# weimengmeng1999/AdapterSIS

Hardware: AMD Instinct MI355X
Metric: training images/sec, ViT-L/14 588^2 adapter fine-tune (higher is better)
Workload: dtype f16; 1 GPU; vit_large/14 frozen + CAViT/CACNN adapters (n_last_blocks=4) + FeatureDecoder, 588x588, batch 12/GPU, reference_exact train.py step (fwd + decoder bwd + all-reduce + SGD), random-init weights; global_batch=12, image_size=588, parallelism=dp1, split_precision_convs=True, split_attn_out=False, precise_level=0, fold_attn_scale=True, fused_qkv=False, dead_cacnn_elided=True, c1_elided=True, ln_fold=True, mx_conv=True, mx_dense=True, conv_halo=True, fuse_cls_up=False, skipped_optimizer_steps=0

## Files before the change

adaptersis_amd/csrc/convhalo.hip:

```cpp
#include <type_traits>
#include "asis_common.h"

namespace {

typedef int v4i_ __attribute__((ext_vector_type(4)));
typedef int v8i_ __attribute__((ext_vector_type(8)));

template <int COUT>
__global__ __launch_bounds__(256, 2) void conv_halo_mx_kernel(const f16* __restrict__ x_hi, const f16* __restrict__ x_mx,
                                                              const f16* __restrict__ w_hi, const f16* __restrict__ w_mx,
                                                              const float* __restrict__ bias, const float* __restrict__ amax_a,
                                                              const float* __restrict__ amax_b, float* __restrict__ out,
                                                              float* __restrict__ stats, int B, int H, int W, int Cin, int TH, int TW, int CT) {
  constexpr int NB = COUT / 16;
  constexpr int MB = 4;
  constexpr int HP = 18 * 18;
  constexpr int HALO = HP * 64;
  constexpr int WT = COUT * 64;
  constexpr int NT = 256;
  __shared__ __attribute__((aligned(16))) f16 lds[HALO + 3 * WT];
  f16* const halo = lds;
  f16* const wbuf0 = lds + HALO;

  const int tid = threadIdx.x, lane = tid & 63;
  const int wid = __builtin_amdgcn_readfirstlane(tid >> 6);
  const int r16 = lane & 15, q16 = lane >> 4;
  int bid = blockIdx.x;
  const int tx_ = bid % TW; bid /= TW;
  const int ty_ = bid % TH;
  const int b = bid / TH;
  const int y0 = ty_ * 16, x0 = tx_ * 16;
  const int64_t img = (int64_t)b * H * W;
  const int K9 = 9 * Cin;
  const int mx_sc = mx_code<f16>(*amax_a, *amax_b);
  const int mx_one = 127;
  const int n0 = blockIdx.y * COUT;
  w_hi += (int64_t)n0 * K9;
  w_mx += (int64_t)n0 * K9;

  f32x4 acc[MB][NB];
#pragma unroll
  for (int i = 0; i < MB; ++i)
#pragma unroll
    for (int j = 0; j < NB; ++j) acc[i][j] = f32x4{0.f, 0.f, 0.f, 0.f};

  const int ngroups = (Cin / 64) * 2;
  constexpr int HLOADS = (HP * 8 + NT - 1) / NT;
  uint4 hreg[HLOADS];
  auto halo_load = [&](int g) {
    const f16* src = (g & 1) ? x_mx : x_hi;
    const int c0 = (g >> 1) * 64;
#pragma unroll
    for (int it = 0; it < HLOADS; ++it) {
      int idx = it * NT + tid;
      idx = idx < HP * 8 ? idx : HP * 8 - 1;
      const int p = idx >> 3, ch = idx & 7;
      const int hy = p / 18, hx = p - hy * 18;
      const int gy = y0 - 1 + hy, gx = x0 - 1 + hx;
      const bool ok = (unsigned)gy < (unsigned)H && (unsigned)gx < (unsigned)W;
      const int cy = ok ? gy : 0, cx = ok ? gx : 0;
      const uint4 v = *reinterpret_cast<const uint4*>(src + ((img + (int64_t)cy * W + cx) * Cin + c0 + ch * 8));
      hreg[it] = ok ? v : make_uint4(0u, 0u, 0u, 0u);
    }
  };
  auto halo_store = [&]() {
#pragma unroll
    for (int it = 0; it < HLOADS; ++it) {
      const int idx = it * NT + tid;
      if (idx < HP * 8) {
        const int p = idx >> 3, ch = idx & 7;
        *reinterpret_cast<uint4*>(halo + p * 64 + ((ch ^ ((p >> 1) & 7)) << 3)) = hreg[it];
      }
    }
  };
  typedef __attribute__((address_space(3))) void* lds_ptr;
  typedef const __attribute__((address_space(1))) void* glb_ptr;
  static_assert(COUT == 64, "two DMA pieces per wave and tap: 4 waves x 2 x 8 rows");
  auto w_dma = [&](int st) {
    const int g = st / 9, tap = st - g * 9;
    const f16* src = (g & 1) ? w_mx : w_hi;
    const int c0 = (g >> 1) * 64;
    f16* dst = wbuf0 + (st % 3) * WT;
#pragma unroll
    for (int i = 0; i < 2; ++i) {
      const int q = wid * 2 + i;
      const int n = q * 8 + (lane >> 3), ch = (lane & 7) ^ ((n >> 1) & 7);
      __builtin_amdgcn_global_load_lds((glb_ptr)(src + (int64_t)n * K9 + tap * Cin + c0 + ch * 8), (lds_ptr)(dst + q * 8 * 64), 16, 0, 0);
    }
  };
  auto mfma_mx = [](f32x4& a, v8i_ x, v8i_ y, int sx, int sy) {
    asm volatile("v_mfma_scale_f32_16x16x128_f8f6f4 %0, %1, %2, %0, %3, %4 op_sel_hi:[0,0,0]" : "+v"(a) : "v"(x), "v"(y), "v"(sx), "v"(sy));
  };

  const int nsteps = ngroups * 9;
  w_dma(0);
  w_dma(1);
  halo_load(0);
  halo_store();
  asm volatile("s_waitcnt vmcnt(0)" ::: "memory");
  __syncthreads();

  int step = 0;
  for (int g = 0; g < ngroups; ++g) {
    const bool next_group = g + 1 < ngroups;
#pragma unroll 1
   for (int tap = 0; tap < 9; ++tap, ++step) {
    if (step + 2 < nsteps) w_dma(step + 2);
    if (tap == 0 && next_group) halo_load(g + 1);
    const f16* wt = wbuf0 + (step % 3) * WT;
    const int ty = tap / 3, tx = tap - ty * 3;
    v8i_ aw[MB];
#pragma unroll
    for (int mb = 0; mb < MB; ++mb) {
      const int p = (wid * MB + mb + ty) * 18 + r16 + tx;
      aw[mb] = __builtin_shufflevector(*reinterpret_cast<const v4i_*>(halo + p * 64 + (((q16) ^ ((p >> 1) & 7)) << 3)),
                                       *reinterpret_cast<const v4i_*>(halo + p * 64 + (((4 + q16) ^ ((p >> 1) & 7)) << 3)), 0, 1, 2, 3, 4, 5, 6, 7);
    }
    auto lo4 = [](v8i_ x) { return __builtin_bit_cast(f16x8, __builtin_shufflevector(x, x, 0, 1, 2, 3)); };
    auto hi4 = [](v8i_ x) { return __builtin_bit_cast(f16x8, __builtin_shufflevector(x, x, 4, 5, 6, 7)); };
    constexpr int NH = 2;
#pragma unroll
    for (int h = 0; h < NB / NH; ++h) {
      v8i_ bw[NH];
#pragma unroll
      for (int k = 0; k < NH; ++k) {
        const int n = (h * NH + k) * 16 + r16;
        bw[k] = __builtin_shufflevector(*reinterpret_cast<const v4i_*>(wt + n * 64 + (((q16) ^ ((n >> 1) & 7)) << 3)),
                                        *reinterpret_cast<const v4i_*>(wt + n * 64 + (((4 + q16) ^ ((n >> 1) & 7)) << 3)), 0, 1, 2, 3, 4, 5, 6, 7);
      }
      if (g & 1) {
        asm volatile("s_waitcnt lgkmcnt(0)" ::: "memory");
#pragma unroll
        for (int k = 0; k < NH; ++k)
#pragma unroll
          for (int mb = 0; mb < MB; ++mb) mfma_mx(acc[mb][h * NH + k], bw[k], aw[mb], mx_sc, mx_one);
      } else {
#pragma unroll
        for (int k = 0; k < NH; ++k)
#pragma unroll
          for (int mb = 0; mb < MB; ++mb) {
            acc[mb][h * NH + k] = T16<f16>::mfma16(lo4(bw[k]), lo4(aw[mb]), acc[mb][h * NH + k]);
            acc[mb][h * NH + k] = T16<f16>::mfma16(hi4(bw[k]), hi4(aw[mb]), acc[mb][h * NH + k]);
          }
      }
    }
    if (step + 1 < nsteps) {
      if (step + 2 >= nsteps) asm volatile("s_waitcnt vmcnt(0)" ::: "memory");
      else if (tap == 0 && next_group) asm volatile("s_waitcnt vmcnt(13)" ::: "memory");
      else asm volatile("s_waitcnt vmcnt(2)" ::: "memory");
    }
    __syncthreads();
    if (tap == 8 && next_group) {
      halo_store();
      __syncthreads();
    }
   }
  }

  float4 s_sum[NB], s_sq[NB];
#pragma unroll
  for (int nb = 0; nb < NB; ++nb) {
    s_sum[nb] = make_float4(0.f, 0.f, 0.f, 0.f);
    s_sq[nb] = make_float4(0.f, 0.f, 0.f, 0.f);
  }
#pragma unroll
  for (int mb = 0; mb < MB; ++mb) {
    const int gy = y0 + wid * MB + mb, gx = x0 + r16;
    const bool ok = gy < H && gx < W;
    float* op = out + (img + (int64_t)(ok ? gy : 0) * W + (ok ? gx : 0)) * CT + n0;
#pragma unroll
    for (int nb = 0; nb < NB; ++nb) {
      const int n = nb * 16 + 4 * q16;
      const float4 bv = bias ? *reinterpret_cast<const float4*>(bias + n0 + n) : make_float4(0.f, 0.f, 0.f, 0.f);
      const float4 v = make_float4(acc[mb][nb][0] + bv.x, acc[mb][nb][1] + bv.y, acc[mb][nb][2] + bv.z, acc[mb][nb][3] + bv.w);
      if (ok) {
        *reinterpret_cast<float4*>(op + n) = v;
        s_sum[nb].x += v.x; s_sum[nb].y += v.y; s_sum[nb].z += v.z; s_sum[nb].w += v.w;
        s_sq[nb].x += v.x * v.x; s_sq[nb].y += v.y * v.y; s_sq[nb].z += v.z * v.z; s_sq[nb].w += v.w * v.w;
      }
    }
  }
  if (stats) {
#pragma unroll
    for (int nb = 0; nb < NB; ++nb)
#pragma unroll
      for (int o = 1; o < 16; o <<= 1) {
        s_sum[nb].x += __shfl_xor(s_sum[nb].x, o, 64); s_sum[nb].y += __shfl_xor(s_sum[nb].y, o, 64);
        s_sum[nb].z += __shfl_xor(s_sum[nb].z, o, 64); s_sum[nb].w += __shfl_xor(s_sum[nb].w, o, 64);
        s_sq[nb].x += __shfl_xor(s_sq[nb].x, o, 64); s_sq[nb].y += __shfl_xor(s_sq[nb].y, o, 64);
        s_sq[nb].z += __shfl_xor(s_sq[nb].z, o, 64); s_sq[nb].w += __shfl_xor(s_sq[nb].w, o, 64);
      }
    float* red = reinterpret_cast<float*>(lds);
    if (r16 == 0) {
#pragma unroll
      for (int nb = 0; nb < NB; ++nb) {
        *reinterpret_cast<float4*>(red + (wid * 2 + 0) * COUT + nb * 16 + 4 * q16) = s_sum[nb];
        *reinterpret_cast<float4*>(red + (wid * 2 + 1) * COUT + nb * 16 + 4 * q16) = s_sq[nb];
      }
    }
    __syncthreads();
    if (tid < 2 * COUT) {
      const int which = tid / COUT, n = tid - which * COUT;
      float s = 0.f;
#pragma unroll
      for (int w4 = 0; w4 < 4; ++w4) s += red[(w4 * 2 + which) * COUT + n];
      stats[((int64_t)blockIdx.x * 2 + which) * CT + n0 + n] = s;
    }
  }
}

}

extern "C" int asis_conv3x3_halo_mx_tiles(int B, int H, int W) { return B * ((H + 15) / 16) * ((W + 15) / 16); }

extern "C" int asis_conv3x3_halo_mx(void* stream, int dtype, const void* x_hi, const void* x_mx, const void* w_hi, const void* w_mx,
                                    const float* bias, const float* amax_a, const float* amax_b, float* out, float* stats, int B,
                                    int H, int W, int Cin, int Cout) {
  ASIS_REQUIRE(x_hi && x_mx && w_hi && w_mx && amax_a && amax_b && out, "asis_conv3x3_halo_mx: null pointer");
  ASIS_REQUIRE(dtype == ASIS_F16, "asis_conv3x3_halo_mx: float16 operands only (the MX correction pass is built for them)");
  ASIS_REQUIRE(B > 0 && H > 0 && W > 0 && Cin > 0 && Cin % 64 == 0 && (Cout == 64 || Cout == 128),
               "asis_conv3x3_halo_mx: Cin=%d must be a multiple of 64, Cout=%d one of 64 / 128", Cin, Cout);
  ASIS_REQUIRE(asis_aligned16(x_hi) && asis_aligned16(x_mx) && asis_aligned16(w_hi) && asis_aligned16(w_mx) && asis_aligned16(out) &&
                   (!bias || asis_aligned16(bias)), "asis_conv3x3_halo_mx: pointers must be 16-byte aligned");
  hipStream_t s = reinterpret_cast<hipStream_t>(stream);
  const int TH = (H + 15) / 16, TW = (W + 15) / 16;
  dim3 grid((unsigned)(B * TH * TW), (unsigned)(Cout / 64)), block(256);
  const f16* xh = reinterpret_cast<const f16*>(x_hi);
  const f16* xm = reinterpret_cast<const f16*>(x_mx);
  const f16* wh = reinterpret_cast<const f16*>(w_hi);
  const f16* wm = reinterpret_cast<const f16*>(w_mx);
  hipLaunchKernelGGL((conv_halo_mx_kernel<64>), grid, block, 0, s, xh, xm, wh, wm, bias, amax_a, amax_b, out, stats, B, H, W, Cin, TH, TW, Cout);
  ASIS_CHECK_LAUNCH("asis_conv3x3_halo_mx");
  return ASIS_OK;
}
```

Baseline: 230.8 img/s.

## Software-pipeline halo conv inner loop with double-buffered A fragments and specialized planes

Restructures the 3x3 halo MX conv main loop: groups are split into compile-time f16 and MX-plane variants so the per-tap branch disappears, the 9 taps are fully unrolled, and A fragments for the next tap are prefetched into a second register set while current MFMAs run. B fragments are loaded incrementally between MFMA batches under sched_barriers, and weight DMA offsets are precomputed once into scalar base plus per-lane offsets. Halo loads always issue (to a dummy address when not needed) with an out-of-bounds bitmask applied at store time, keeping vmcnt accounting uniform. The costs are higher register pressure from double-buffered fragments and heavier code from unrolling, which could cut occupancy below the two blocks per CU the kernel is launched for.

New measurement: 232.3 img/s, median of 6. About the same (+0.6%).

```diff
diff --git a/adaptersis_amd/csrc/convhalo.hip b/adaptersis_amd/csrc/convhalo.hip
--- a/adaptersis_amd/csrc/convhalo.hip
+++ b/adaptersis_amd/csrc/convhalo.hip
@@ -47,116 +47,153 @@
   const int ngroups = (Cin / 64) * 2;
   constexpr int HLOADS = (HP * 8 + NT - 1) / NT;
   uint4 hreg[HLOADS];
-  auto halo_load = [&](int g) {
+  uint32_t hmask = 0;
+  auto halo_load = [&](int g, bool live) {
     const f16* src = (g & 1) ? x_mx : x_hi;
     const int c0 = (g >> 1) * 64;
+    int t = tid;
+    asm volatile("" : "+v"(t));
+    hmask = 0;
 #pragma unroll
     for (int it = 0; it < HLOADS; ++it) {
-      int idx = it * NT + tid;
+      int idx = it * NT + t;
       idx = idx < HP * 8 ? idx : HP * 8 - 1;
       const int p = idx >> 3, ch = idx & 7;
       const int hy = p / 18, hx = p - hy * 18;
       const int gy = y0 - 1 + hy, gx = x0 - 1 + hx;
       const bool ok = (unsigned)gy < (unsigned)H && (unsigned)gx < (unsigned)W;
       const int cy = ok ? gy : 0, cx = ok ? gx : 0;
-      const uint4 v = *reinterpret_cast<const uint4*>(src + ((img + (int64_t)cy * W + cx) * Cin + c0 + ch * 8));
-      hreg[it] = ok ? v : make_uint4(0u, 0u, 0u, 0u);
+      const int64_t off = (img + (int64_t)cy * W + cx) * Cin + c0 + ch * 8;
+      hreg[it] = *reinterpret_cast<const uint4*>(live ? src + off : x_hi);
+      hmask |= (ok ? 1u : 0u) << it;
+      __builtin_amdgcn_sched_barrier(0);
     }
   };
   auto halo_store = [&]() {
+    int t = tid;
+    asm volatile("" : "+v"(t));
 #pragma unroll
     for (int it = 0; it < HLOADS; ++it) {
-      const int idx = it * NT + tid;
+      const int idx = it * NT + t;
       if (idx < HP * 8) {
         const int p = idx >> 3, ch = idx & 7;
-        *reinterpret_cast<uint4*>(halo + p * 64 + ((ch ^ ((p >> 1) & 7)) << 3)) = hreg[it];
+        *reinterpret_cast<uint4*>(halo + p * 64 + ((ch ^ ((p >> 1) & 7)) << 3)) = (hmask >> it) & 1u ? hreg[it] : make_uint4(0u, 0u, 0u, 0u);
       }
     }
   };
   typedef __attribute__((address_space(3))) void* lds_ptr;
   typedef const __attribute__((address_space(1))) void* glb_ptr;
   static_assert(COUT == 64, "two DMA pieces per wave and tap: 4 waves x 2 x 8 rows");
+  uint32_t woff[2];
+#pragma unroll
+  for (int i = 0; i < 2; ++i) {
+    const int n = (wid * 2 + i) * 8 + (lane >> 3), ch = (lane & 7) ^ ((n >> 1) & 7);
+    woff[i] = (uint32_t)(n * K9 + ch * 8) * 2u;
+  }
   auto w_dma = [&](int st) {
     const int g = st / 9, tap = st - g * 9;
-    const f16* src = (g & 1) ? w_mx : w_hi;
-    const int c0 = (g >> 1) * 64;
+    uint64_t sb = reinterpret_cast<uint64_t>(((g & 1) ? w_mx : w_hi) + tap * Cin + (g >> 1) * 64);
+    asm volatile("" : "+s"(sb));
+    const char* src = reinterpret_cast<const char*>(sb);
     f16* dst = wbuf0 + (st % 3) * WT;
 #pragma unroll
-    for (int i = 0; i < 2; ++i) {
-      const int q = wid * 2 + i;
-      const int n = q * 8 + (lane >> 3), ch = (lane & 7) ^ ((n >> 1) & 7);
-      __builtin_amdgcn_global_load_lds((glb_ptr)(src + (int64_t)n * K9 + tap * Cin + c0 + ch * 8), (lds_ptr)(dst + q * 8 * 64), 16, 0, 0);
-    }
+    for (int i = 0; i < 2; ++i)
+      __builtin_amdgcn_global_load_lds((glb_ptr)(src + woff[i]), (lds_ptr)(dst + (wid * 2 + i) * 8 * 64), 16, 0, 0);
   };
   auto mfma_mx = [](f32x4& a, v8i_ x, v8i_ y, int sx, int sy) {
     asm volatile("v_mfma_scale_f32_16x16x128_f8f6f4 %0, %1, %2, %0, %3, %4 op_sel_hi:[0,0,0]" : "+v"(a) : "v"(x), "v"(y), "v"(sx), "v"(sy));
   };
 
-  const int nsteps = ngroups * 9;
+  auto frag = [&](const f16* base, int row, int q) {
+    return __builtin_shufflevector(*reinterpret_cast<const v4i_*>(base + row * 64 + (((q) ^ ((row >> 1) & 7)) << 3)),
+                                   *reinterpret_cast<const v4i_*>(base + row * 64 + (((4 + q) ^ ((row >> 1) & 7)) << 3)), 0, 1, 2, 3, 4, 5, 6, 7);
+  };
+  auto lane_rq = [&](int& r, int& q) {
+    r = r16;
+    q = q16;
+    asm volatile("" : "+v"(r), "+v"(q));
+  };
+  auto a_read = [&](v8i_ (&aw)[MB], int tap) {
+    const int ty = tap / 3, tx = tap - ty * 3;
+    int r, q;
+    lane_rq(r, q);
+#pragma unroll
+    for (int mb = 0; mb < MB; ++mb) aw[mb] = frag(halo, (wid * MB + mb + ty) * 18 + r + tx, q);
+  };
+  auto lo4 = [](v8i_ x) { return __builtin_bit_cast(f16x8, __builtin_shufflevector(x, x, 0, 1, 2, 3)); };
+  auto hi4 = [](v8i_ x) { return __builtin_bit_cast(f16x8, __builtin_shufflevector(x, x, 4, 5, 6, 7)); };
+  auto barrier = [&]() {
+    __builtin_amdgcn_s_barrier();
+    asm volatile("" ::: "memory");
+  };
+
   w_dma(0);
   w_dma(1);
-  halo_load(0);
+  halo_load(0, true);
   halo_store();
-  asm volatile("s_waitcnt vmcnt(0)" ::: "memory");
-  __syncthreads();
-
-  int step = 0;
-  for (int g = 0; g < ngroups; ++g) {
+  asm volatile("s_waitcnt vmcnt(0) lgkmcnt(0)" ::: "memory");
+  barrier();
+
+  auto run_group = [&](auto plane, int g) {
+    constexpr bool MX = decltype(plane)::value;
     const bool next_group = g + 1 < ngroups;
+    const int step0 = g * 9;
+    v8i_ aw[2][MB];
+    a_read(aw[0], 0);
+#pragma unroll
+    for (int tap = 0; tap < 9; ++tap) {
+      if (next_group || tap < 7) w_dma(step0 + tap + 2);
+      if (tap == 0) {
+        asm volatile("" ::: "memory");
+        __builtin_amdgcn_sched_barrier(0);
+        halo_load(g + 1, next_group);
+      }
+      const f16* wt = wbuf0 + (tap % 3) * WT;
+      v8i_ bw[2];
+      int rb, qb;
+      lane_rq(rb, qb);
+      bw[0] = frag(wt, rb, qb);
+      bw[1] = frag(wt, 16 + rb, qb);
+      if (tap < 8) a_read(aw[(tap + 1) & 1], tap + 1);
+      __builtin_amdgcn_sched_barrier(0);
+      const v8i_(&a)[MB] = aw[tap & 1];
+#pragma unroll
+      for (int nb = 0; nb < NB; ++nb) {
+        const v8i_ b8 = bw[nb & 1];
+        if constexpr (MX) {
+#pragma unroll
+          for (int mb = 0; mb < MB; ++mb) mfma_mx(acc[mb][nb], b8, a[mb], mx_sc, mx_one);
+        } else {
+#pragma unroll
+          for (int mb = 0; mb < MB; ++mb) acc[mb][nb] = T16<f16>::mfma16(lo4(b8), lo4(a[mb]), acc[mb][nb]);
+#pragma unroll
+          for (int mb = 0; mb < MB; ++mb) acc[mb][nb] = T16<f16>::mfma16(hi4(b8), hi4(a[mb]), acc[mb][nb]);
+        }
+        __builtin_amdgcn_sched_barrier(0);
+        if (nb + 2 < NB) {
+          bw[nb & 1] = frag(wt, (nb + 2) * 16 + rb, qb);
+          __builtin_amdgcn_sched_barrier(0);
+        }
+      }
+      if (!next_group && tap >= 7) asm volatile("s_waitcnt vmcnt(0) lgkmcnt(0)" ::: "memory");
+      else if (tap < 2) asm volatile("s_waitcnt vmcnt(13) lgkmcnt(0)" ::: "memory");
+      else asm volatile("s_waitcnt vmcnt(2) lgkmcnt(0)" ::: "memory");
+      barrier();
+      if (tap == 8 && next_group) {
+        halo_store();
+        asm volatile("s_waitcnt lgkmcnt(0)" ::: "memory");
+        barrier();
+      }
+    }
+  };
 #pragma unroll 1
-   for (int tap = 0; tap < 9; ++tap, ++step) {
-    if (step + 2 < nsteps) w_dma(step + 2);
-    if (tap == 0 && next_group) halo_load(g + 1);
-    const f16* wt = wbuf0 + (step % 3) * WT;
-    const int ty = tap / 3, tx = tap - ty * 3;
-    v8i_ aw[MB];
-#pragma unroll
-    for (int mb = 0; mb < MB; ++mb) {
-      const int p = (wid * MB + mb + ty) * 18 + r16 + tx;
-      aw[mb] = __builtin_shufflevector(*reinterpret_cast<const v4i_*>(halo + p * 64 + (((q16) ^ ((p >> 1) & 7)) << 3)),
-                                       *reinterpret_cast<const v4i_*>(halo + p * 64 + (((4 + q16) ^ ((p >> 1) & 7)) << 3)), 0, 1, 2, 3, 4, 5, 6, 7);
-    }
-    auto lo4 = [](v8i_ x) { return __builtin_bit_cast(f16x8, __builtin_shufflevector(x, x, 0, 1, 2, 3)); };
-    auto hi4 = [](v8i_ x) { return __builtin_bit_cast(f16x8, __builtin_shufflevector(x, x, 4, 5, 6, 7)); };
-    constexpr int NH = 2;
-#pragma unroll
-    for (int h = 0; h < NB / NH; ++h) {
-      v8i_ bw[NH];
-#pragma unroll
-      for (int k = 0; k < NH; ++k) {
-        const int n = (h * NH + k) * 16 + r16;
-        bw[k] = __builtin_shufflevector(*reinterpret_cast<const v4i_*>(wt + n * 64 + (((q16) ^ ((n >> 1) & 7)) << 3)),
-                                        *reinterpret_cast<const v4i_*>(wt + n * 64 + (((4 + q16) ^ ((n >> 1) & 7)) << 3)), 0, 1, 2, 3, 4, 5, 6, 7);
-      }
-      if (g & 1) {
-        asm volatile("s_waitcnt lgkmcnt(0)" ::: "memory");
-#pragma unroll
-        for (int k = 0; k < NH; ++k)
-#pragma unroll
-          for (int mb = 0; mb < MB; ++mb) mfma_mx(acc[mb][h * NH + k], bw[k], aw[mb], mx_sc, mx_one);
-      } else {
-#pragma unroll
-        for (int k = 0; k < NH; ++k)
-#pragma unroll
-          for (int mb = 0; mb < MB; ++mb) {
-            acc[mb][h * NH + k] = T16<f16>::mfma16(lo4(bw[k]), lo4(aw[mb]), acc[mb][h * NH + k]);
-            acc[mb][h * NH + k] = T16<f16>::mfma16(hi4(bw[k]), hi4(aw[mb]), acc[mb][h * NH + k]);
-          }
-      }
-    }
-    if (step + 1 < nsteps) {
-      if (step + 2 >= nsteps) asm volatile("s_waitcnt vmcnt(0)" ::: "memory");
-      else if (tap == 0 && next_group) asm volatile("s_waitcnt vmcnt(13)" ::: "memory");
-      else asm volatile("s_waitcnt vmcnt(2)" ::: "memory");
-    }
-    __syncthreads();
-    if (tap == 8 && next_group) {
-      halo_store();
-      __syncthreads();
-    }
-   }
-  }
-
+  for (int g = 0; g < ngroups; g += 2) {
+    run_group(std::false_type{}, g);
+    run_group(std::true_type{}, g + 1);
+  }
+
+  int re = r16, qe = q16, te = tid;
+  asm volatile("" : "+v"(re), "+v"(qe), "+v"(te));
   float4 s_sum[NB], s_sq[NB];
 #pragma unroll
   for (int nb = 0; nb < NB; ++nb) {
@@ -165,12 +202,12 @@
   }
 #pragma unroll
   for (int mb = 0; mb < MB; ++mb) {
-    const int gy = y0 + wid * MB + mb, gx = x0 + r16;
+    const int gy = y0 + wid * MB + mb, gx = x0 + re;
     const bool ok = gy < H && gx < W;
     float* op = out + (img + (int64_t)(ok ? gy : 0) * W + (ok ? gx : 0)) * CT + n0;
 #pragma unroll
     for (int nb = 0; nb < NB; ++nb) {
-      const int n = nb * 16 + 4 * q16;
+      const int n = nb * 16 + 4 * qe;
       const float4 bv = bias ? *reinterpret_cast<const float4*>(bias + n0 + n) : make_float4(0.f, 0.f, 0.f, 0.f);
       const float4 v = make_float4(acc[mb][nb][0] + bv.x, acc[mb][nb][1] + bv.y, acc[mb][nb][2] + bv.z, acc[mb][nb][3] + bv.w);
       if (ok) {
@@ -191,16 +228,16 @@
         s_sq[nb].z += __shfl_xor(s_sq[nb].z, o, 64); s_sq[nb].w += __shfl_xor(s_sq[nb].w, o, 64);
       }
     float* red = reinterpret_cast<float*>(lds);
-    if (r16 == 0) {
+    if (re == 0) {
 #pragma unroll
       for (int nb = 0; nb < NB; ++nb) {
-        *reinterpret_cast<float4*>(red + (wid * 2 + 0) * COUT + nb * 16 + 4 * q16) = s_sum[nb];
-        *reinterpret_cast<float4*>(red + (wid * 2 + 1) * COUT + nb * 16 + 4 * q16) = s_sq[nb];
+        *reinterpret_cast<float4*>(red + (wid * 2 + 0) * COUT + nb * 16 + 4 * qe) = s_sum[nb];
+        *reinterpret_cast<float4*>(red + (wid * 2 + 1) * COUT + nb * 16 + 4 * qe) = s_sq[nb];
       }
     }
     __syncthreads();
-    if (tid < 2 * COUT) {
-      const int which = tid / COUT, n = tid - which * COUT;
+    if (te < 2 * COUT) {
+      const int which = te / COUT, n = te - which * COUT;
       float s = 0.f;
 #pragma unroll
       for (int w4 = 0; w4 < 4; ++w4) s += red[(w4 * 2 + which) * COUT + n];
```
